# RuanJohn/Mava

Measured on AMD Instinct MI355X. Metric: env-steps/sec (whole node), ff_mappo RWARE tiny-4ag, higher is better.
Workload: dtype f32 via 2 x f16 split operands on the MFMA (3 products, f32 accumulate); 1 GPU; ff_mappo RWARE tiny-4ag-shaped synthetic obs, 4096 envs/GPU (update_batch_size=1 x num_envs=4096), rollout_length=128, ppo_epochs=4, num_minibatches=2, agents=4, obs=70/264, actions=5, one step = one PPO update = 524288 env-steps per GPU; parallelism=dp1

## Files before the change

### include/mava_hip.h

```cpp
#ifndef MAVA_HIP_H
#define MAVA_HIP_H

#include <stddef.h>
#include <stdint.h>

#ifdef __cplusplus
extern "C" {
#endif

typedef struct ihipStream_t* mava_stream_t;

const char* mava_last_error(void);
int mava_abi_version(void);

typedef struct mava_ctx mava_ctx;
enum {
  MAVA_CTX_MATMUL_MODE = 0,
  MAVA_CTX_CRITIC_AGGREGATION = 1,
  MAVA_CTX_GAE_VARIANT = 2,
  MAVA_CTX_POLICY_VARIANT = 3,
  MAVA_CTX_H2_LAUNCHES = 4,
  MAVA_CTX_TRAIN_VARIANT = 5,
  MAVA_CTX_W8_LAUNCHES = 6,
  MAVA_CTX_W1_SPLIT_FRESH = 7,
  MAVA_CTX_EXACT_TILES = 8,
  MAVA_CTX_X16_LAUNCHES = 9,
  MAVA_CTX_X16_W8_LAUNCHES = 10,
  MAVA_CTX_W8_DEFER_LAUNCHES = 11,
  MAVA_CTX_W8_AHEAD_LAUNCHES = 12
};
int mava_ctx_create(mava_ctx** out);
int mava_ctx_destroy(mava_ctx* ctx);
int mava_ctx_set(mava_ctx* ctx, int key, long value);
int mava_ctx_get(const mava_ctx* ctx, int key, long* value);

int mava_gae_f32(const mava_ctx* ctx, const float* reward, const float* value, const uint8_t* done,
                 const float* last_val, const uint8_t* last_done, int T, int N, float gamma,
                 float lambda, float* adv, float* tgt, mava_stream_t s);

int mava_permutation_i32(long n, uint64_t seed, uint64_t counter, int32_t* out, mava_stream_t s);
int mava_permutation_batched_i32(long n, uint64_t seed, uint64_t counter, int n_perm, int32_t* out, long out_stride,
                                 mava_stream_t s);

int mava_clip_adam(float* p, const float* g, float* m, float* v, int32_t* count,
                   const int* seg_off, const float* seg_lr, int n_seg, float grad_scale,
                   float max_norm, int decay, int steps_per_update, int num_updates, float b1,
                   float b2, float eps, const float* loss_sums, float vf_coef, float ent_coef,
                   float* metrics_out, mava_stream_t s);

size_t mava_ppo_finish_workspace_bytes(int Pa, int Pc);
int mava_ppo_finish_f32(mava_ctx* ctx, const float* slab_a, long stride_a, const float* slab_c, long stride_c, int n_slab,
                        int Pa, int Pc, float* g, float* p, float* m, float* v, int32_t* count, float lr_a, float lr_c,
                        float grad_scale, float max_norm, int decay, int steps_per_update, int num_updates, float b1,
                        float b2, float eps, float vf_coef, float ent_coef, float* metrics_out, int critic_din,
                        void* workspace, size_t workspace_bytes, mava_stream_t s);

int mava_slab_reduce_f32(const float* slab, int n_slab, long slab_stride, int n, int accumulate,
                         float* out, mava_stream_t s);

int mava_slab_reduce2_f32(const float* slab, int n_slab, long slab_stride, int n_main,
                          float* out_main, int n_tail, float* out_tail, int accumulate,
                          mava_stream_t s);
// ... 324 lines not shown
```

### mava_amd/_lib.py

```python
from __future__ import annotations

import ctypes as C
import os
from typing import Optional

import torch

_HERE = os.path.dirname(os.path.abspath(__file__))
LIB_PATH = os.environ.get("MAVA_LIB_PATH") or os.path.join(_HERE, "libmavahip.so")

_lib: Optional[C.CDLL] = None


class MavaHipError(RuntimeError):
    pass


vp = C.c_void_p
i32 = C.c_int
u32 = C.c_uint32
u64 = C.c_uint64
f32 = C.c_float
lng = C.c_long

# ... 106 lines not shown
             "mava_transformer_param_count_continuous": C.c_long}


def declared_symbols():
    return sorted(set(_SIGNATURES) | set(_RESTYPES))


def lib() -> C.CDLL:
    global _lib
    if _lib is None:
        if not os.path.exists(LIB_PATH):
            raise MavaHipError(
                f"{LIB_PATH} is missing: build it with `python -m mava_amd.build` "
                "(hipcc --offload-arch=gfx950). There is no CPU fallback."
            )
        _lib = C.CDLL(LIB_PATH)
        _lib.mava_last_error.restype = C.c_char_p
        _lib.mava_last_error.argtypes = []
        for name, args in _SIGNATURES.items():
            fn = getattr(_lib, name)
            fn.argtypes = args
            fn.restype = _RESTYPES.get(name, C.c_int)
    return _lib


class Ctx:

    MATMUL_MODE, CRITIC_AGGREGATION, GAE_VARIANT, POLICY_VARIANT, H2_LAUNCHES, TRAIN_VARIANT, W8_LAUNCHES, W1_SPLIT_FRESH = 0, 1, 2, 3, 4, 5, 6, 7
    EXACT_TILES = 8
    X16_LAUNCHES = 9
    X16_W8_LAUNCHES = 10
    W8_DEFER_LAUNCHES = 11
    W8_AHEAD_LAUNCHES = 12

    def __init__(self, matmul_mode: str = "f32", critic_aggregation: bool = True):
        if matmul_mode not in ("f32", "f16x2"):
            raise ValueError(f"matmul_mode must be 'f16x2' or 'f32', got {matmul_mode!r}")
        h = C.c_void_p()
        check(lib().mava_ctx_create(C.byref(h)), "mava_ctx_create")
        self.handle: Optional[int] = h.value
        self.set(self.MATMUL_MODE, 1 if matmul_mode == "f16x2" else 0)
        self.set(self.CRITIC_AGGREGATION, int(bool(critic_aggregation)))

    def set(self, key: int, value: int) -> None:
        check(lib().mava_ctx_set(self.handle, key, int(value)), "mava_ctx_set")

    def get(self, key: int) -> int:
        out = C.c_long()
        check(lib().mava_ctx_get(self.handle, key, C.byref(out)), "mava_ctx_get")
        return int(out.value)

    @property
    def matmul_mode(self) -> str:
        return "f16x2" if self.get(self.MATMUL_MODE) == 1 else "f32"

    @property
    def h2_launches(self) -> int:
        return self.get(self.H2_LAUNCHES)

    def close(self) -> None:
        if getattr(self, "handle", None) is not None and _lib is not None:
            _lib.mava_ctx_destroy(self.handle)
        self.handle = None

    def __del__(self):
        try:
# ... 41 lines not shown
```

### mava_amd/csrc/api.cpp

```cpp
#include <stdarg.h>
#include <stdio.h>
#include <string.h>

#include "common.h"
#include "ctx.h"

static thread_local char g_err[512] = "";

void mava_set_error(const char* fmt, ...) {
  va_list ap;
  va_start(ap, fmt);
  vsnprintf(g_err, sizeof(g_err), fmt, ap);
  va_end(ap);
}

extern "C" const char* mava_last_error(void) { return g_err; }

extern "C" int mava_abi_version(void) { return 4; }

enum { CTX_MATMUL_MODE = 0, CTX_CRITIC_AGGREGATION = 1, CTX_GAE_VARIANT = 2, CTX_POLICY_VARIANT = 3, CTX_H2_LAUNCHES = 4, CTX_TRAIN_VARIANT = 5, CTX_W8_LAUNCHES = 6, CTX_W1_SPLIT_FRESH = 7, CTX_EXACT_TILES = 8, CTX_X16_LAUNCHES = 9, CTX_X16_W8_LAUNCHES = 10, CTX_W8_DEFER_LAUNCHES = 11, CTX_W8_AHEAD_LAUNCHES = 12 };
static int ctx_counter_word(int key) {
  return key == CTX_W8_AHEAD_LAUNCHES ? 4 : key == CTX_W8_DEFER_LAUNCHES ? 3 : key == CTX_X16_W8_LAUNCHES ? 2 : key == CTX_X16_LAUNCHES ? 1 : 0;
}

extern "C" int mava_ctx_create(mava_ctx** out) {
  MAVA_ARG_CHECK(out != nullptr, 0, "mava_ctx_create: null output pointer");
  mava_ctx* c = new mava_ctx();
  c->matmul_mode = 0;
  c->critic_aggregation = 1;
  c->gae_variant = 0;
  c->policy_variant = 0;
  c->h2_launches = 0;
  c->train_variant = 0;
  c->w8_launches = 0;
  c->w1_split[0] = c->w1_split[1] = nullptr;
  for (int i = 0; i < 2; ++i) {
    c->w1_fresh[i] = 0;
    c->w1_key_params[i] = nullptr;
    c->w1_key_din[i] = c->w1_key_steps[i] = 0;
  }
  c->exact_tiles = nullptr;
  *out = c;
  return MAVA_OK;
}

extern "C" int mava_ctx_destroy(mava_ctx* c) {
  if (c == nullptr) return MAVA_OK;
  for (int i = 0; i < 2; ++i)
    if (c->w1_split[i] != nullptr) (void)hipFree(c->w1_split[i]);
  if (c->exact_tiles != nullptr) (void)hipFree(c->exact_tiles);
  delete c;
  return MAVA_OK;
}

extern "C" int mava_ctx_set(mava_ctx* c, int key, long value) {
  MAVA_ARG_CHECK(c != nullptr, 0, "mava_ctx_set: null context");
  switch (key) {
    case CTX_MATMUL_MODE:
      MAVA_ARG_CHECK(value == 0 || value == 1, 1, "mava_ctx_set: matmul mode %ld (0 = exact f32, 1 = f16x2)", value);
      c->matmul_mode = (int)value;
      c->w1_fresh[0] = c->w1_fresh[1] = 0;
      return MAVA_OK;
    case CTX_CRITIC_AGGREGATION: c->critic_aggregation = value ? 1 : 0; return MAVA_OK;
    case CTX_GAE_VARIANT: c->gae_variant = (int)value; return MAVA_OK;
    case CTX_POLICY_VARIANT: c->policy_variant = (int)value; return MAVA_OK;
    case CTX_H2_LAUNCHES: c->h2_launches = value; return MAVA_OK;
    case CTX_TRAIN_VARIANT: c->train_variant = (int)value; return MAVA_OK;
    case CTX_W8_LAUNCHES: c->w8_launches = value; return MAVA_OK;
    case CTX_W1_SPLIT_FRESH:
      MAVA_ARG_CHECK(value == 0, 1, "mava_ctx_set: MAVA_CTX_W1_SPLIT_FRESH can only be cleared (0) by the caller");
      c->w1_fresh[0] = c->w1_fresh[1] = 0;
      return MAVA_OK;
    case CTX_EXACT_TILES:
      MAVA_ARG_CHECK(value == 0, 1, "mava_ctx_set: MAVA_CTX_EXACT_TILES can only be reset (0) by the caller");
      if (c->exact_tiles != nullptr) {
        MAVA_HIP_CHECK(hipDeviceSynchronize());
        MAVA_HIP_CHECK(hipMemset(c->exact_tiles, 0, sizeof(unsigned long long)));
      }
      return MAVA_OK;
    case CTX_X16_LAUNCHES:
    case CTX_X16_W8_LAUNCHES:
    case CTX_W8_DEFER_LAUNCHES:
    case CTX_W8_AHEAD_LAUNCHES:
      MAVA_ARG_CHECK(value == 0, 1, "mava_ctx_set: MAVA_CTX_X16_LAUNCHES / _W8_LAUNCHES / MAVA_CTX_W8_DEFER_LAUNCHES / _AHEAD_LAUNCHES can only be reset (0) by the caller");
      if (c->exact_tiles != nullptr) {
        MAVA_HIP_CHECK(hipDeviceSynchronize());
        MAVA_HIP_CHECK(hipMemset(c->exact_tiles + ctx_counter_word(key), 0, sizeof(unsigned long long)));
      }
      return MAVA_OK;
    default: mava_set_error("mava_ctx_set: unknown key %d", key); return MAVA_EARG(2);
  }
}

extern "C" int mava_ctx_get(const mava_ctx* c, int key, long* value) {
  MAVA_ARG_CHECK(c != nullptr && value != nullptr, 0, "mava_ctx_get: null argument");
  switch (key) {
    case CTX_MATMUL_MODE: *value = c->matmul_mode; return MAVA_OK;
    case CTX_CRITIC_AGGREGATION: *value = c->critic_aggregation; return MAVA_OK;
    case CTX_GAE_VARIANT: *value = c->gae_variant; return MAVA_OK;
    case CTX_POLICY_VARIANT: *value = c->policy_variant; return MAVA_OK;
    case CTX_H2_LAUNCHES: *value = c->h2_launches; return MAVA_OK;
    case CTX_TRAIN_VARIANT: *value = c->train_variant; return MAVA_OK;
    case CTX_W8_LAUNCHES: *value = c->w8_launches; return MAVA_OK;
    case CTX_W1_SPLIT_FRESH: *value = c->w1_fresh[1]; return MAVA_OK;
    case CTX_EXACT_TILES:
    case CTX_X16_LAUNCHES:
    case CTX_X16_W8_LAUNCHES:
    case CTX_W8_DEFER_LAUNCHES:
    case CTX_W8_AHEAD_LAUNCHES: {
      unsigned long long n = 0;
      if (c->exact_tiles != nullptr) {
        MAVA_HIP_CHECK(hipDeviceSynchronize());
        MAVA_HIP_CHECK(hipMemcpy(&n, c->exact_tiles + ctx_counter_word(key), sizeof(n), hipMemcpyDeviceToHost));
      }
      *value = (long)n;
      return MAVA_OK;
    }
    default: mava_set_error("mava_ctx_get: unknown key %d", key); return MAVA_EARG(2);
  }
}
```

### mava_amd/csrc/ppo_train_h2.hip

```cpp
#include "h2_core.h"
#include "ppo_train_task.h"
#include "ctx.h"

#include <type_traits>

#ifndef MAVA_GW_DEPTH
#define MAVA_GW_DEPTH 0
#endif
#define GW_DEPTH MAVA_GW_DEPTH
#ifndef MAVA_GW_DEPTH_WIDE
#define MAVA_GW_DEPTH_WIDE 0
#endif
#ifndef MAVA_P1_EARLY_HALVES
#define MAVA_P1_EARLY_HALVES 2
#endif
#ifndef MAVA_P1_EARLY_RING
#define MAVA_P1_EARLY_RING 3
#endif

namespace {

using namespace h2;

constexpr int STATS_BLOCKS = 128;

#ifdef MAVA_STAMPS
#define STAMP_DECL unsigned long long st_prev = __builtin_readcyclecounter(), st_acc[16] = {0, 0, 0, 0, 0, 0, 0, 0, 0, 0, 0, 0, 0, 0, 0, 0};
#define STAMP(i)                                                    \
  do {                                                              \
    __builtin_amdgcn_sched_barrier(0);                              \
    const unsigned long long st_now = __builtin_readcyclecounter(); \
    st_acc[i] += st_now - st_prev;                                  \
    st_prev = st_now;                                               \
    __builtin_amdgcn_sched_barrier(0);                              \
  } while (0)
#else
#define STAMP_DECL
#define STAMP(i)
#endif

struct H2Layout {
  int h1, dz2, dz1, w2, xs, xs_plane, xs_row, dy, yp, agg, small, relu, end;
};

template <int NO, int S1, bool WIDE>
H2Layout make_h2_layout(bool actor) {
  constexpr int KT1 = (S1 + 1) / 2;
  H2Layout L;
  L.h1 = 0;
  L.dz2 = L.h1 + IMG_BYTES;
  L.dz1 = L.dz2 + IMG_BYTES;
  L.w2 = L.dz1 + IMG_BYTES;
  L.xs = L.w2 + 4 * IMG_BYTES;
  L.xs_row = 2 * 32 * KT1 + 16;
  L.xs_plane = 32 * L.xs_row;
  L.dy = L.xs + (WIDE ? 1 : 2) * 2 * L.xs_plane;
  L.yp = actor ? L.dz2 : L.dz1;
  L.agg = L.dy + (actor ? 2 * DY_PLANE : 0);
  L.small = L.agg + 8 * 33 * 4;
  L.small = (L.small + 15) & ~15;
  L.relu = L.small + (128 + 32 + 16 + 128) * 4;
  L.end = L.relu + (WIDE ? 256 * 4 : 0);
  return L;
}
constexpr int W2_PLANE = 128 * SW_ROW;
constexpr int W1_RING = 3;

template <int STEPS>
__global__ __launch_bounds__(256) void pack_w1_kernel(const float* __restrict__ P, int din, uint4* __restrict__ out, float scale) {
  pack_w1_body<STEPS>(P, din, out, threadIdx.x, scale);
}

template <int NO, int S1, bool ACTOR, bool WIDE, int XV, int ROLE, bool X16 = false>
__device__ __forceinline__ void h2_body(const TrainTask& tk, const H2Layout& L, const uint4* __restrict__ w1p, u8* lds) {
  static_assert(!WIDE || S1 % W1_RING == 0, "WIDE: S1 must be a multiple of the W1 ring depth");
  static_assert((ROLE == 0) == !WIDE, "roles 1 / 2 belong to WIDE launches");
  static_assert(!X16 || (WIDE && !ACTOR), "the f16 copy of x is read by the wide critic only");
  constexpr bool CHAIN = ROLE != 2, LOADER = ROLE != 1;
#if defined(MAVA_NO_W2_RESIDENT) || defined(MAVA_W2_RESIDENT_P4)
  constexpr bool W2_RESIDENT = false;
#else
  constexpr bool W2_RESIDENT = !WIDE && NO <= 16;
#endif
#ifdef MAVA_W2_RESIDENT_P4
  constexpr bool W2_RES4 = !WIDE && ACTOR && NO <= 16;
#else
  constexpr bool W2_RES4 = false;
#endif
  constexpr int NTHR = WIDE ? 512 : 256;
  constexpr float WS = ACTOR ? 1.0f : W_SCALE_CRITIC, WU = 1.0f / WS;
  constexpr int KT1 = (S1 + 1) / 2;
  u8* const H1I = lds + L.h1;
  u8* const DZ2I = lds + L.dz2;
  u8* const DZ1I = lds + L.dz1;
  u8* const H2I = lds + L.dz1;
  u8* const W2I = lds + L.w2;
  u8* const DYI = lds + L.dy;
  float* const YP = reinterpret_cast<float*>(lds + L.yp);
  float* const AGG = reinterpret_cast<float*>(lds + L.agg);
  float* const B2s = reinterpret_cast<float*>(lds + L.small);
  float* const B3s = B2s + 128;
  float* const misc = B3s + 32;
  float* const W3s = misc + 16;
  uint32_t* const RELU1 = reinterpret_cast<uint32_t*>(lds + L.relu);
  constexpr bool VERSIONED = WIDE && !ACTOR;
  constexpr int P1_EARLY = VERSIONED ? MAVA_P1_EARLY_HALVES * (S1 / 2) : 0;
  static_assert(MAVA_P1_EARLY_HALVES >= 0 && MAVA_P1_EARLY_HALVES <= 2, "P1_EARLY is 0, S1 / 2 or S1");
  constexpr bool EARLY = P1_EARLY > 0, EARLY_ALL = EARLY && P1_EARLY == S1;
  const int xs_row = L.xs_row, xs_plane = L.xs_plane;

  int tid = threadIdx.x & 255;
  int lane = tid & 63, w = tid >> 6, h = lane >> 5, r = lane & 31;
  int srow = tid >> 3, l8 = tid & 7;
  const int din = tk.din, no = tk.no;
  const long R = (!ACTOR && tk.agg > 1) ? (long)tk.Rb : (long)tk.Rb * tk.A;
  const float invR = 1.0f / (float)((long)tk.Rb * tk.A);
  constexpr int NPC = (32 * KT1 / XV + 7) / 8;
  constexpr int NR = NPC * XV;

  for (int i = threadIdx.x * 16; i < L.end; i += NTHR * 16) *reinterpret_cast<uint4*>(lds + i) = make_uint4(0, 0, 0, 0);
  __syncthreads();
  const float* const P = tk.params;
  const int oW2 = mlp_off_w2(din), oW3 = mlp_off_w3(din);
  if (CHAIN) {
    if (tid < 128) B2s[tid] = P[mlp_off_b2(din) + tid];
    if (tid < no) B3s[tid] = P[mlp_off_b3(din, no) + tid];
    if (!ACTOR && tid < 128) W3s[tid] = P[oW3 + tid];
    if (tid < (WIDE ? 32 : 64)) {
      const int b = tid >> 5, row = tid & 31;
      *reinterpret_cast<_Float16*>(lds + L.xs + b * 2 * xs_plane + row * xs_row + 2 * din) = (_Float16)1.0f;
    }
    {
      const int n = tid & 127, k0 = 64 * (tid >> 7);
      float carry = 0.0f;
#pragma unroll 8
      for (int k = k0; k < k0 + 64; ++k) {
        _Float16 x0, x1;
        split1_carry(P[oW2 + k * MLP_H + n] * WS, carry, x0, x1);
        const int o = sw_off(k, n >> 3) + 2 * (n & 7);
        *reinterpret_cast<_Float16*>(W2I + o) = x0;
        *reinterpret_cast<_Float16*>(W2I + W2_PLANE + o) = x1;
// ... 260 lines not shown
        cursor_advance(cs);
      }
      if (CHAIN) {
#pragma unroll
        for (int q = 0; q < NP; ++q) cursor_gather(cl[q], pl_next[q], al_next[q]);
#pragma unroll
        for (int q = 0; q < NP; ++q) cursor_advance(cl[q]);
      }
    }
  }
  __syncthreads();

  SwRow rowB = sw_row(r, h);
  SwTr trS = sw_tr(lane);
  const int i16 = lane & 15, tq = i16 >> 2, tp = i16 & 3, g1 = (lane >> 4) & 1;
  int trX = (8 * h + tq) * xs_row + 2 * (16 * g1 + 4 * tp);
  const int trD = (8 * h + tq) * DY_ROW + 2 * (16 * g1 + 4 * tp);
  SwRow w2row = sw_row(32 * w + r, h);
  int buf = 0;
  Frag w2r[(W2_RESIDENT || W2_RES4) ? 8 : 1];
  if constexpr (W2_RESIDENT) {
#pragma unroll
    for (int s = 0; s < 8; ++s) w2r[s] = sw_read_tr(W2I, W2_PLANE, trS, s, w);
  }
  if constexpr (W2_RES4) {
#pragma unroll
    for (int s = 0; s < 8; ++s) w2r[s] = sw_read_row(W2I, W2_PLANE, w2row, s);
  }

  STAMP_DECL
  bool exact = false;
  unsigned n_exact = 0;
  constexpr int ER = MAVA_P1_EARLY_RING, SB = S1 - P1_EARLY;
  constexpr int GB = P1_EARLY / 9, GC = GB + (P1_EARLY * 7) / 18;
  f32x16 eC, eL;
  Frag W1e[(EARLY && LOADER) ? ER : 1];
  auto early_fill = [&]() __attribute__((always_inline)) {
#pragma unroll
    for (int g = 0; g < ER && g < P1_EARLY; ++g) W1e[g] = w1_fetch(SB + g);
  };
  auto early_steps = [&](auto g0_tag, auto g1_tag, const u8* xsi) __attribute__((always_inline)) {
    constexpr int G0 = decltype(g0_tag)::value, G1 = decltype(g1_tag)::value;
    if constexpr (G0 < G1) {
      half8 xh = *reinterpret_cast<const half8*>(xsi + r * xs_row + 16 * h + 32 * (SB + G0));
#pragma unroll
      for (int g = G0; g < G1; ++g) {
        const half8 b = xh;
        if (g + 1 < G1) xh = *reinterpret_cast<const half8*>(xsi + r * xs_row + 16 * h + 32 * (SB + g + 1));
        if (g == 0 || SB + g == S1 / 2) {
#pragma unroll
          for (int q = 0; q < 16; ++q) {
            if (SB + g < S1 / 2) eC[q] = 0.0f; else eL[q] = 0.0f;
          }
        }
        if (SB + g < S1 / 2) {
          eC = __builtin_amdgcn_mfma_f32_32x32x16_f16(W1e[g % ER].lo, b, eC, 0, 0, 0);
          eC = __builtin_amdgcn_mfma_f32_32x32x16_f16(W1e[g % ER].hi, b, eC, 0, 0, 0);
        } else {
          eL = __builtin_amdgcn_mfma_f32_32x32x16_f16(W1e[g % ER].lo, b, eL, 0, 0, 0);
          eL = __builtin_amdgcn_mfma_f32_32x32x16_f16(W1e[g % ER].hi, b, eL, 0, 0, 0);
        }
        if (g >= 1 && g - 1 + ER < P1_EARLY) W1e[(g - 1) % ER] = w1_fetch(SB + g - 1 + ER);
        __builtin_amdgcn_sched_barrier(0);
      }
    }
  };
  uint32_t xrow_keep = 0;
  auto tile_body = [&](auto exact_tag) __attribute__((always_inline)) {
    constexpr bool EXACT = decltype(exact_tag)::value;
    static_assert(!EXACT || VERSIONED, "the exact-input loop belongs to the wide critic");
    constexpr bool XE = EXACT && EARLY;
    STAMP(14);
    const bool valid = (it * 32 + r) < R;
    const long itn = it + gridDim.x;
    const bool have_next = itn < ntiles;
    if constexpr (EXACT && LOADER && !X16) {
      if (tid == 0) xflag[tpar ^ 1] = 0u;
    }
    uint32_t xrow_next = LOADER ? stage_row(ps_next, as_next) : 0u;
    uint32_t fr_next[NP];
#pragma unroll
    for (int q = 0; q < NP; ++q) fr_next[q] = CHAIN ? ((uint32_t)pl_next[q] * Au + al_next[q]) : 0u;
    if (LOADER) asm volatile("" : "+v"(xrow_next));
    if (CHAIN) {
#pragma unroll
      for (int q = 0; q < NP; ++q) asm volatile("" : "+v"(fr_next[q]));
    }
    const u8* const XSI = lds + L.xs + (EXACT ? tpar : 2 * buf) * xs_plane;
    if constexpr (XE && LOADER) xrow_keep = xrow_next;

    f32x16 acc;
    uint32_t relu1 = 0;
    if constexpr (WIDE) asm volatile("" : "+v"(w1p_lane));
    if constexpr ((CHAIN || WIDE) && !(XE && (LOADER || EARLY_ALL))) {
#pragma unroll
    for (int q = 0; q < 16; ++q) acc[q] = 0.0f;
    if constexpr (WIDE && !CHAIN) {
#pragma unroll
      for (int s = 0; s < NW1; ++s) W1f[s] = w1_fetch(S_LO + s);
    }
    Frag xb;
    xb.hi = *reinterpret_cast<const half8*>(XSI + r * xs_row + 16 * h + 32 * S_LO);
    if constexpr (!EXACT) xb.lo = *reinterpret_cast<const half8*>(XSI + xs_plane + r * xs_row + 16 * h + 32 * S_LO);
#pragma unroll
    for (int j = 0; j < RL; ++j) {
      const Frag b = xb;
      if (j + 1 < RL) {
        xb.hi = *reinterpret_cast<const half8*>(XSI + r * xs_row + 16 * h + 32 * (S_LO + j + 1));
        if constexpr (!EXACT) xb.lo = *reinterpret_cast<const half8*>(XSI + xs_plane + r * xs_row + 16 * h + 32 * (S_LO + j + 1));
      }
      if constexpr (EXACT) {
        acc = __builtin_amdgcn_mfma_f32_32x32x16_f16(W1f[j % NW1].lo, b.hi, acc, 0, 0, 0);
        acc = __builtin_amdgcn_mfma_f32_32x32x16_f16(W1f[j % NW1].hi, b.hi, acc, 0, 0, 0);
      } else {
        acc = mfma3(W1f[j % NW1], b, acc);
      }
      if (WIDE) {
        if (j >= 1 && j - 1 + W1_RING < RL) W1f[(j - 1) % NW1] = w1_fetch(S_LO + j - 1 + W1_RING);
      }
      __builtin_amdgcn_sched_barrier(0);
    }
    }
    if constexpr (XE && EARLY_ALL && LOADER) {
#pragma unroll
      for (int q = 0; q < 16; ++q) {
        acc[q] = fmaxf((eC[q] + eL[q]) * WU, 0.0f);
        relu1 |= (acc[q] > 0.0f) ? (1u << q) : 0u;
      }
      __builtin_amdgcn_sched_barrier(0);
      issue(have_next ? xrow_next : 0u);
      __builtin_amdgcn_sched_barrier(0);
      half4 ph[4], pl[4];
      sw_write_image(H1I, r, w, h, acc, ph, pl);
      RELU1[tid] = relu1;
    }
    if constexpr (WIDE && !(XE && EARLY_ALL)) {
      float4* const xch = reinterpret_cast<float4*>(DZ2I) + (w * 4) * 64 + lane;
      if constexpr (LOADER) {
        if constexpr (XE) {
          acc = eL;
          issue(have_next ? xrow_next : 0u);
        }
#pragma unroll
        for (int g = 0; g < 4; ++g) xch[g * 64] = make_float4(acc[4 * g], acc[4 * g + 1], acc[4 * g + 2], acc[4 * g + 3]);
      }
      __syncthreads();
      if constexpr (CHAIN) {
#pragma unroll
        for (int g = 0; g < 4; ++g) {
          const float4 v = xch[g * 64];
          acc[4 * g] += v.x; acc[4 * g + 1] += v.y; acc[4 * g + 2] += v.z; acc[4 * g + 3] += v.w;
        }
      }
    }
    if constexpr (CHAIN && !(XE && EARLY_ALL)) {
    STAMP(0);
#pragma unroll
    for (int q = 0; q < 16; ++q) {
      acc[q] = fmaxf(ACTOR ? acc[q] : acc[q] * WU, 0.0f);
      relu1 |= (acc[q] > 0.0f) ? (1u << q) : 0u;
    }
    {
      half4 ph[4], pl[4];
      sw_write_image(H1I, r, w, h, acc, ph, pl);
// ... 30 lines not shown
      }
    } else if (have_next) {
      if (LOADER && !WIDE) issue(xrow_next);
      const bool more = itn + gridDim.x < ntiles;
      if (more) {
        if (LOADER) {
          cursor_gather(cs, ps_next, as_next);
          cursor_advance(cs);
        }
        if (CHAIN) {
          Cursor c_old[NP];
#pragma unroll
          for (int q = 0; q < NP; ++q) { c_old[q] = cl[q]; cursor_advance(cl[q]); }
          __builtin_amdgcn_sched_barrier(0);
#pragma unroll
          for (int q = 0; q < NP; ++q) cursor_gather(c_old[q], pl_next[q], al_next[q]);
        }
      }
      if (CHAIN) {
#pragma unroll
        for (int q = 0; q < NP; ++q) load_row((long)fr_next[q], n_act[q], n_f0[q], n_f1[q], n_m[q]);
      }
    }
    if constexpr (WIDE && CHAIN && !(XE && EARLY_ALL)) {
      __builtin_amdgcn_sched_barrier(0);
#pragma unroll
      for (int s2 = 0; s2 < NW1; ++s2) W1f[s2] = w1_fetch(S_LO + s2);
      __builtin_amdgcn_sched_barrier(0);
    }
    STAMP(2);
    __syncthreads();
    STAMP(3);
    if constexpr (XE && LOADER) {
      commit_hi(lds + L.xs + (tpar ^ 1) * xs_plane, tpar ^ 1);
      early_fill();
    }
    if constexpr (XE && EARLY_ALL && CHAIN) relu1 = RELU1[tid];

    f32x16 h2;
    uint32_t relu2 = 0;
    if constexpr (CHAIN) {
#pragma unroll
    for (int q = 0; q < 16; ++q) h2[q] = B2s[32 * w + (q & 3) + 8 * (q >> 2) + 4 * h] * WS;
    {
      Frag an;
      if constexpr (!W2_RESIDENT) an = sw_read_tr(W2I, W2_PLANE, trS, 0, w);
      Frag bn = sw_read_row(H1I, SW_PLANE, rowB, 0);
#pragma unroll
      for (int s = 0; s < 8; ++s) {
        const Frag a = W2_RESIDENT ? w2r[s] : an, b = bn;
        if (s + 1 < 8) {
          if constexpr (!W2_RESIDENT) an = sw_read_tr(W2I, W2_PLANE, trS, s + 1, w);
          bn = sw_read_row(H1I, SW_PLANE, rowB, s + 1);
        }
        h2 = mfma3(a, b, h2);
        __builtin_amdgcn_sched_barrier(0);
      }
    }
    STAMP(4);
#pragma unroll
    for (int q = 0; q < 16; ++q) {
      h2[q] = fmaxf(ACTOR ? h2[q] : h2[q] * WU, 0.0f);
      relu2 |= (h2[q] > 0.0f) ? (1u << q) : 0u;
    }
    if (!ACTOR) {
      float4 w3g[4];
#pragma unroll
      for (int g = 0; g < 4; ++g) w3g[g] = *reinterpret_cast<const float4*>(W3s + 32 * w + 4 * h + 8 * g);
// ... 1 lines not shown
#pragma unroll
      for (int q = 0; q < 16; ++q) {
        const float4 t = w3g[q >> 2];
        const float w3 = (q & 3) == 0 ? t.x : (q & 3) == 1 ? t.y : (q & 3) == 2 ? t.z : t.w;
        part = fmaf(h2[q], w3, part);
      }
      part += __shfl_xor(part, 32, 64);
      if (h == 0) YP[(w * 32 + r) * (NO + 1)] = part;
    } else {
      half4 ph[4], pl[4];
      sw_write_image(H2I, r, w, h, h2, ph, pl);
      f32x16 yacc;
#pragma unroll
      for (int q = 0; q < 16; ++q) yacc[q] = 0.0f;
#pragma unroll
      for (int s = 0; s < 2; ++s) {
        Frag b;
        b.hi = __builtin_shufflevector(ph[2 * s], ph[2 * s + 1], 0, 1, 2, 3, 4, 5, 6, 7);
        b.lo = __builtin_shufflevector(pl[2 * s], pl[2 * s + 1], 0, 1, 2, 3, 4, 5, 6, 7);
        yacc = mfma3(W3h[s], b, yacc);
      }
#pragma unroll
      for (int q = 0; q < 16; ++q) {
        const int o = (q & 3) + 8 * (q >> 2) + 4 * h;
        if ((q & 3) + 8 * (q >> 2) < NO) {
          if (o < NO) YP[(w * 32 + r) * (NO + 1) + o] = yacc[q] * W3_UNSCALE;
        }
      }
    }
    }
    STAMP(5);
    __syncthreads();
    STAMP(6);
    if constexpr (XE && LOADER) early_steps(std::integral_constant<int, 0>{}, std::integral_constant<int, GB>{}, lds + L.xs + (tpar ^ 1) * xs_plane);
    if constexpr (EXACT && LOADER && !XE) {
      commit_hi(lds + L.xs + (tpar ^ 1) * xs_plane, tpar ^ 1);
    }

    f32x16 dz;
    float dy0 = 0.0f;
    if constexpr (CHAIN) {
    if (ACTOR) {
      const float lo_c = 1.0f - tk.clip_eps, hi_c = 1.0f + tk.clip_eps;
#pragma unroll
      for (int q = 0; q < NP; ++q) {
        const int row = loss_row(q);
        const bool rvalid = (it * 32 + row) < R;
        const float* yp = YP + row * (NO + 1) + lo;
        const float y = (((yp[0] + yp[32 * (NO + 1)]) + yp[2 * 32 * (NO + 1)]) + yp[3 * 32 * (NO + 1)]) + B3s[lo];
        const bool legal = (lo < no) && (r_m[q] != 0u);
        const float z = legal ? y : -FLT_MAX;
        auto fmax_op = [](float a, float b) { return fmaxf(a, b); };
        auto add_op = [](float a, float b) { return a + b; };
        const float mx = group_allreduce<NO>(z, fmax_op);
        const float se = group_allreduce<NO>(expf(z - mx), add_op);
        const float logp = (mx == -FLT_MAX) ? ((lo < no) ? -logf((float)no) : -FLT_MAX) : z - (mx + logf(se));
        const float pr = expf(logp);
        const float ent = group_allreduce<NO>((pr > 0.0f) ? -(pr * logp) : 0.0f, add_op);
        const int act = r_act[q];
        const float lp = group_allreduce<NO>((lo == act) ? logp : 0.0f, add_op);
        const float gae = (r_f1[q] - adv_mean) * adv_rstd;
        const float ratio = expf(lp - r_f0[q]);
        const float rc = fminf(fmaxf(ratio, lo_c), hi_c);
        const float l1 = ratio * gae, l2 = rc * gae;
        const float pg = -fminf(l1, l2);
        const bool inside = (ratio >= lo_c) && (ratio <= hi_c);
// ... 131 lines not shown
      if constexpr (!W2_RES4) an = sw_read_row(W2I, W2_PLANE, w2row, 0);
      Frag bn = sw_read_row(DZ2I, SW_PLANE, rowB, 0);
#pragma unroll
      for (int s = 0; s < 8; ++s) {
        const Frag a = W2_RES4 ? w2r[s] : an, b = bn;
        if (s + 1 < 8) {
          if constexpr (!W2_RES4) an = sw_read_row(W2I, W2_PLANE, w2row, s + 1);
          bn = sw_read_row(DZ2I, SW_PLANE, rowB, s + 1);
        }
        acc = mfma3(a, b, acc);
        __builtin_amdgcn_sched_barrier(0);
      }
#pragma unroll
      for (int q = 0; q < 16; ++q) acc[q] = ((relu1 >> q) & 1u) ? (ACTOR ? acc[q] : acc[q] * WU) : 0.0f;
      half4 ph[4], pl[4];
      sw_write_image(DZ1I, r, w, h, acc, ph, pl);
    }
    if constexpr (!WIDE) {
      if constexpr (!X16) {
        if (have_next) stage_commit(false_type{}, false_type{}, lds + L.xs + (buf ^ 1) * 2 * xs_plane, xr, 0);
      }
    }
    if constexpr (XE && LOADER) early_steps(std::integral_constant<int, GC>{}, std::integral_constant<int, P1_EARLY>{}, lds + L.xs + (tpar ^ 1) * xs_plane);
    STAMP(10);
    if constexpr (!WIDE) do_gw2();
    STAMP(11);
    __syncthreads();
    STAMP(12);
    if constexpr (WIDE && CHAIN) do_gw2();
    if constexpr (LOADER) {
      constexpr int NPR = 2 * KT1;
      constexpr int D1 = WIDE ? MAVA_GW_DEPTH_WIDE : GW_DEPTH;
      if constexpr (EXACT) {
#pragma unroll
        for (int s = 0; s < 2; ++s) {
          const Frag b = sw_read_tr(DZ1I, SW_PLANE, trS, s, w);
#pragma unroll
          for (int t = 0; t < KT1; ++t) {
            const half8 a = read_tr8(XSI + trX + 16 * s * xs_row + 2 * (32 * t), xs_row);
            const f32x16 c = __builtin_amdgcn_mfma_f32_32x32x16_f16(a, b.lo, gW1[t], 0, 0, 0);
            gW1[t] = __builtin_amdgcn_mfma_f32_32x32x16_f16(a, b.hi, c, 0, 0, 0);
            if (t & 1) __builtin_amdgcn_sched_barrier(0);
          }
        }
      } else if constexpr (D1 > 0) {
        constexpr int DP = D1 < NPR ? D1 : NPR;
        const Frag b0 = sw_read_tr(DZ1I, SW_PLANE, trS, 0, w), b1 = sw_read_tr(DZ1I, SW_PLANE, trS, 1, w);
        Frag a[DP > 0 ? DP : 1];
#pragma unroll
        for (int i = 0; i < DP; ++i) a[i] = read_tr_frag(XSI + trX + 16 * (i / KT1) * xs_row + 2 * (32 * (i % KT1)), xs_plane, xs_row);
#pragma unroll
        for (int i = 0; i < NPR; ++i) {
          const Frag cur = a[i % (DP > 0 ? DP : 1)];
          if (i + DP < NPR)
            a[i % (DP > 0 ? DP : 1)] = read_tr_frag(XSI + trX + 16 * ((i + DP) / KT1) * xs_row + 2 * (32 * ((i + DP) % KT1)), xs_plane, xs_row);
          gW1[i % KT1] = mfma3(cur, (i / KT1) ? b1 : b0, gW1[i % KT1]);
          __builtin_amdgcn_sched_barrier(0);
        }
      } else {
#pragma unroll
        for (int s = 0; s < 2; ++s) {
          const Frag b = sw_read_tr(DZ1I, SW_PLANE, trS, s, w);
#pragma unroll
          for (int t = 0; t < KT1; ++t) {
            const Frag a = read_tr_frag(XSI + trX + 16 * s * xs_row + 2 * (32 * t), xs_plane, xs_row);
            gW1[t] = mfma3(a, b, gW1[t]);
            if (t & 1) __builtin_amdgcn_sched_barrier(0);
          }
        }
      }
    }
    STAMP(13);
    if constexpr (WIDE) {
      __syncthreads();
      if constexpr (EXACT) {
        if constexpr (!X16) exact = __builtin_amdgcn_readfirstlane((int)xflag[tpar ^ 1]) == 0;
        ++n_exact;
      } else {
        if constexpr (LOADER && !X16) {
          stage_commit(false_type{}, false_type{}, lds + L.xs, xr, 0);
        }
        __syncthreads();
      }
    }
    if constexpr (CHAIN) {
#pragma unroll
      for (int q = 0; q < NP; ++q) { r_act[q] = n_act[q]; r_f0[q] = n_f0[q]; r_f1[q] = n_f1[q]; r_m[q] = n_m[q]; }
    }
  };
  if constexpr (VERSIONED) {
    exact = X16 || (__builtin_amdgcn_readfirstlane((int)xflag[0]) == 0 && tk.force_xlo == 0);
    if (exact && it < ntiles) {
      if (CHAIN && tid < 32) *reinterpret_cast<_Float16*>(lds + L.xs + xs_plane + tid * xs_row + 2 * din) = (_Float16)1.0f;
    }
    if constexpr (EARLY && LOADER) {
      early_fill();
      early_steps(std::integral_constant<int, 0>{}, std::integral_constant<int, P1_EARLY>{}, lds + L.xs);
    }
    if constexpr (X16) {
      for (; it < ntiles; it += gridDim.x, tpar ^= 1) tile_body(true_type{});
    } else {
    for (; it < ntiles && exact; it += gridDim.x, tpar ^= 1) tile_body(true_type{});
    asm volatile("" : "+v"(tid), "+v"(lane), "+v"(w), "+v"(h), "+v"(r), "+v"(trS.b0), "+v"(trS.b1), "+v"(trS.q64));
    if constexpr (LOADER) asm volatile("" : "+v"(srow), "+v"(l8), "+v"(trX));
    if constexpr (CHAIN) asm volatile("" : "+v"(rowB.base), "+v"(rowB.hx), "+v"(w2row.base), "+v"(w2row.hx));
    if (n_exact != 0 && it < ntiles) {
      if constexpr (LOADER) {
        if constexpr (EARLY) {
          asm volatile("" : "+v"(xrow_keep));
          stage_issue(xrow_keep, xr);
        }
        stage_commit(false_type{}, false_type{}, lds + L.xs, xr, 0);
      }
      if (CHAIN && tid < 32) *reinterpret_cast<_Float16*>(lds + L.xs + xs_plane + tid * xs_row + 2 * din) = (_Float16)0.0f;
      __syncthreads();
    }
    if constexpr (EARLY_ALL && CHAIN) {
#pragma unroll
      for (int s = 0; s < NW1; ++s) W1f[s] = w1_fetch(S_LO + s);
    }
    }
  }
  if constexpr (!X16) {
    for (; it < ntiles; it += gridDim.x, buf ^= (WIDE ? 0 : 1)) tile_body(false_type{});
  }
#ifdef MAVA_STAMPS
  if (tk.stamps != nullptr && blockIdx.x == 0 && lane == 0) {
    for (int i = 0; i < 16; ++i) tk.stamps[((ROLE == 2 ? 4 : 0) + w) * 16 + i] = st_acc[i];
  }
#endif

  __syncthreads();
  if constexpr (VERSIONED && CHAIN) {
    if (tid == 0 && tk.exact_tiles != nullptr) atomicAdd(tk.exact_tiles, (unsigned long long)n_exact);
    if constexpr (X16) {
      if (tid == 0 && blockIdx.x == 0 && tk.x16_launches != nullptr) atomicAdd(tk.x16_launches, 1ull);
    }
  }
  float* slab = tk.slab + (long)blockIdx.x * tk.slab_stride;
  const int oB2 = mlp_off_b2(din), oB3 = mlp_off_b3(din, no);
  const int Pn = mlp_param_count(din, no);
  if constexpr (LOADER) {
#pragma unroll
    for (int t = 0; t < KT1; ++t)
#pragma unroll
      for (int q = 0; q < 16; ++q) {
        const int k = mlp_feat(t, q, h);
        if (k <= din) slab[k * MLP_H + 32 * w + r] = gW1[t][q] * invR;
      }
  }
  if constexpr (CHAIN) {
#pragma unroll
    for (int t = 0; t < 4; ++t)
#pragma unroll
      for (int q = 0; q < 16; ++q) slab[oW2 + mlp_feat(t, q, h) * MLP_H + 32 * w + r] = gW2[t][q] * invR;
#pragma unroll
    for (int q = 0; q < 16; ++q) {
      float v = ab2[q];
#pragma unroll
      for (int m = 1; m < 32; m <<= 1) v += __shfl_xor(v, m, 64);
      if (r == 0) slab[oB2 + 32 * w + (q & 3) + 8 * (q >> 2) + 4 * h] = v * invR;
    }
  }
  float* red = reinterpret_cast<float*>(lds + L.h1);
  if constexpr (!CHAIN) {
    __syncthreads();
  } else if (ACTOR) {
#pragma unroll
    for (int q = 0; q < 16; ++q) {
      const int o = (q & 3) + 8 * (q >> 2) + 4 * h;
      if (o < no) slab[oW3 + (32 * w + r) * no + o] = gW3[q] * invR;
// ... 18 lines not shown
    for (int q = 0; q < 16; ++q) {
      float v = aW3r[q];
#pragma unroll
      for (int m = 1; m < 32; m <<= 1) v += __shfl_xor(v, m, 64);
      if (r == 0) slab[oW3 + 32 * w + (q & 3) + 8 * (q >> 2) + 4 * h] = v * invR;
    }
    float v = ab3, l = loss_a;
    for (int o = 32; o > 0; o >>= 1) {
      v += __shfl_down(v, o, 64);
      l += __shfl_down(l, o, 64);
    }
    if (lane == 0) { red[2 * w] = v; red[2 * w + 1] = l; }
    __syncthreads();
    if (tid == 0) {
      slab[oB3] = (((red[0] + red[2]) + red[4]) + red[6]) * invR;
      slab[Pn] = ((red[1] + red[3]) + red[5]) + red[7];
      slab[Pn + 1] = 0.0f;
    }
  }
}

template <int NO, int S1, bool ACTOR, bool WIDE, int XV>
__global__ __launch_bounds__(WIDE ? 512 : 256, WIDE ? 2 : 1) void ppo_train_h2_kernel(TrainTask tk, H2Layout L,
                                                                                     const uint4* __restrict__ w1p) {
  extern __shared__ __attribute__((aligned(16))) u8 lds[];
  if constexpr (WIDE) {
    constexpr bool X16_CAPABLE = !ACTOR && XV == 4;
    bool x16 = false;
    if constexpr (X16_CAPABLE) {
      if (tk.x16_valid != nullptr) x16 = __builtin_amdgcn_readfirstlane((int)*tk.x16_valid) == 1;
    }
    if (X16_CAPABLE && x16) {
      if constexpr (X16_CAPABLE) {
        if (threadIdx.x < 256) {
          h2_body<NO, S1, ACTOR, WIDE, XV, 1, true>(tk, L, w1p, lds);
        } else {
          h2_body<NO, S1, ACTOR, WIDE, XV, 2, true>(tk, L, w1p, lds);
        }
      }
    } else if (threadIdx.x < 256) {
      h2_body<NO, S1, ACTOR, WIDE, XV, 1>(tk, L, w1p, lds);
    } else {
      h2_body<NO, S1, ACTOR, WIDE, XV, 2>(tk, L, w1p, lds);
    }
  } else {
    h2_body<NO, S1, ACTOR, WIDE, XV, 0>(tk, L, w1p, lds);
  }
}

int ctx_counters(mava_ctx* ctx, hipStream_t s) {
  if (ctx->exact_tiles == nullptr) {
    void* word = nullptr;
    MAVA_HIP_CHECK(hipMalloc(&word, 5 * sizeof(unsigned long long)));
    ctx->exact_tiles = static_cast<unsigned long long*>(word);
    MAVA_HIP_CHECK(hipMemsetAsync(word, 0, 5 * sizeof(unsigned long long), s));
  }
  return MAVA_OK;
}

template <int NO, int S1, bool ACTOR, bool WIDE, int XV>
int launch_h2(mava_ctx* ctx, const TrainTask& tk, int n_slab, hipStream_t s) {
  const H2Layout L = make_h2_layout<NO, S1, WIDE>(ACTOR);
  MAVA_ARG_CHECK(L.end <= 163840, 8, "ppo_train_h2: %d bytes of LDS exceed the 160 KiB of a CU", L.end);
  static bool attr_set = false;
  if (!attr_set) {
    MAVA_HIP_CHECK(hipFuncSetAttribute((const void*)ppo_train_h2_kernel<NO, S1, ACTOR, WIDE, XV>,
                                       hipFuncAttributeMaxDynamicSharedMemorySize, L.end));
    attr_set = true;
  }
  const uint4* w1p = nullptr;
  if (WIDE) {
    void*& slot = ctx->w1_split[ACTOR ? 0 : 1];
    if (slot == nullptr) MAVA_HIP_CHECK(hipMalloc(&slot, W1_SPLIT_BYTES));
    uint4* const buf = static_cast<uint4*>(slot);
    const int kind = ACTOR ? 0 : 1;
    int& fresh = ctx->w1_fresh[kind];
    const bool keyed = ctx->w1_key_params[kind] == tk.params && ctx->w1_key_din[kind] == tk.din && ctx->w1_key_steps[kind] == S1;
    if (!(fresh && keyed)) {
      hipLaunchKernelGGL((pack_w1_kernel<S1>), dim3(1), dim3(256), 0, s, tk.params, tk.din, buf, ACTOR ? 1.0f : W_SCALE_CRITIC);
      MAVA_LAUNCH_CHECK();
    }
    fresh = 0;
    w1p = buf;
    const int rc = ctx_counters(ctx, s);
    if (rc != MAVA_OK) return rc;
  }
  TrainTask tkl = tk;
  tkl.exact_tiles = WIDE ? ctx->exact_tiles : nullptr;
  const bool x16_ok = WIDE && !ACTOR && XV == 4 && tk.x16 != nullptr && tk.x16_valid != nullptr && tk.din % 8 == 0 &&
                      (uintptr_t)tk.x16 % 16 == 0 && tk.force_xlo == 0 && (tk.x16_ld == 0 || tk.x16_ld == tk.din);
  if (!x16_ok) { tkl.x16 = nullptr; tkl.x16_valid = nullptr; }
  tkl.x16_launches = x16_ok ? ctx->exact_tiles + 1 : nullptr;
  g_train_last_instance = train_instance_id(2, ACTOR, false, WIDE, NO, S1, XV);
  hipLaunchKernelGGL((ppo_train_h2_kernel<NO, S1, ACTOR, WIDE, XV>), dim3(n_slab), dim3(WIDE ? 512 : 256), L.end, s, tkl, L,
                     w1p);
  MAVA_LAUNCH_CHECK();
  return MAVA_OK;
}

template <int NO, int S1, bool ACTOR, bool WIDE>
int dispatch_xv(mava_ctx* ctx, const TrainTask& tk, int n_slab, hipStream_t s) {
  const uintptr_t a = (uintptr_t)tk.x;
  if constexpr (WIDE) {
    if (tk.din % 4 == 0 && a % 16 == 0) return launch_h2<NO, S1, ACTOR, WIDE, 4>(ctx, tk, n_slab, s);
  } else {
    if (tk.din % 2 == 0 && a % 8 == 0) return launch_h2<NO, S1, ACTOR, WIDE, 2>(ctx, tk, n_slab, s);
  }
  return launch_h2<NO, S1, ACTOR, WIDE, 1>(ctx, tk, n_slab, s);
}

template <int NO, bool ACTOR>
int dispatch_s1(mava_ctx* ctx, const TrainTask& tk, int n_slab, hipStream_t s) {
  const int s1 = (tk.din + 1 + 15) / 16;
  switch (s1) {
#ifndef MAVA_FAST_BUILD
    case 1: return dispatch_xv<NO, 1, ACTOR, false>(ctx, tk, n_slab, s);
    case 2: return dispatch_xv<NO, 2, ACTOR, false>(ctx, tk, n_slab, s);
    case 3: return dispatch_xv<NO, 3, ACTOR, false>(ctx, tk, n_slab, s);
    case 4: return dispatch_xv<NO, 4, ACTOR, false>(ctx, tk, n_slab, s);
    case 6: return dispatch_xv<NO, 6, ACTOR, false>(ctx, tk, n_slab, s);
    case 7: case 8: case 9: case 10: case 11: case 12: return dispatch_xv<NO, 12, ACTOR, true>(ctx, tk, n_slab, s);
#endif
    case 5: return dispatch_xv<NO, 5, ACTOR, false>(ctx, tk, n_slab, s);
    case 13: case 14: case 15: case 16: case 17: case 18: return dispatch_xv<NO, 18, ACTOR, true>(ctx, tk, n_slab, s);
    default: return 1;
  }
}

}

static int h2_dispatch(mava_ctx* ctx, const TrainTask& tk, int n_slab, bool actor, hipStream_t s) {
  if (actor) {
    if (tk.action_f != nullptr) return 1;
    if (tk.no <= 8) return dispatch_s1<8, true>(ctx, tk, n_slab, s);
#ifndef MAVA_FAST_BUILD
    if (tk.no <= 16) return dispatch_s1<16, true>(ctx, tk, n_slab, s);
    return dispatch_s1<32, true>(ctx, tk, n_slab, s);
#else
    return 1;
#endif
  }
  return dispatch_s1<1, false>(ctx, tk, n_slab, s);
}

int mava_train_h2_launch(mava_ctx* ctx, const TrainTask& tk_in, int n_slab, bool actor, hipStream_t s) {
  TrainTask tk = tk_in;
  tk.force_xlo = (ctx->train_variant & 2) != 0;
  tk.no_defer = (ctx->train_variant & 4) != 0;
  tk.no_ahead = (ctx->train_variant & 8) != 0;
  if ((ctx->train_variant & 1) == 0) {
    if (tk.x16 != nullptr && tk.x16_valid != nullptr) {
      const int rcc = ctx_counters(ctx, s);
      if (rcc != MAVA_OK) return rcc;
      tk.x16_launches = ctx->exact_tiles + 2;
      tk.defer_launches = ctx->exact_tiles + 3;
      tk.ahead_launches = ctx->exact_tiles + 4;
    }
    const int rc8 = mava_train_w8_launch(tk, n_slab, actor, s);
    if (rc8 <= 0) {
      if (rc8 == 0) { ++ctx->h2_launches; ++ctx->w8_launches; }
      return rc8;
    }
  }
  const int rc = h2_dispatch(ctx, tk, n_slab, actor, s);
  if (rc == 0) ++ctx->h2_launches;
  return rc;
}
```

### mava_amd/csrc/ppo_train_task.h

```cpp
#pragma once
#include <stdint.h>

#include "common.h"

struct TrainTask {
  const float* params;
  const float* x;
  int din, no, xshare, xv;
  int A;
  int agg;
  const int32_t* idx;
  long idx_base;
  int Rb;
  const uint8_t* mask;
  const int32_t* action;
  const float* action_f;
  uint32_t seed_lo, seed_hi, ent_step, row_offset;
  float min_scale;
  const float* old_logp;
  const float* adv;
  const double* stats;
  const float* old_value;
  const float* targets;
  float clip_eps, ent_coef, vf_coef;
  float* slab;
  long slab_stride;
  unsigned long long* stamps;
  int force_xlo;
  unsigned long long* exact_tiles;
  const _Float16* x16;
  const uint32_t* x16_valid;
  unsigned long long* x16_launches;
  int x16_ld;
  int no_defer;
  unsigned long long* defer_launches;
  int no_ahead;
  unsigned long long* ahead_launches;
};

struct mava_ctx;
int mava_train_w8_launch(const TrainTask& tk, int n_slab, bool actor, hipStream_t s);
int mava_train_h2_launch(mava_ctx* ctx, const TrainTask& tk, int n_slab, bool actor, hipStream_t s);

extern int g_train_last_instance;
constexpr int train_instance_id(int family, bool actor, bool cont, bool wide, int no, int k, int xv) {
  return family * 1000000 + ((actor ? 1 : 0) + (cont ? 2 : 0) + (wide ? 4 : 0)) * 100000 + no * 1000 + k * 10 + xv;
}
```

Before: 88.09 million env-steps/s.

## Defer tail of exact dW1 products into next tile's loader phase for wide critic

```diff
diff --git a/include/mava_hip.h b/include/mava_hip.h
--- a/include/mava_hip.h
+++ b/include/mava_hip.h
@@ -27,7 +27,8 @@
   MAVA_CTX_X16_LAUNCHES = 9,
   MAVA_CTX_X16_W8_LAUNCHES = 10,
   MAVA_CTX_W8_DEFER_LAUNCHES = 11,
-  MAVA_CTX_W8_AHEAD_LAUNCHES = 12
+  MAVA_CTX_W8_AHEAD_LAUNCHES = 12,
+  MAVA_CTX_WIDE_DEFER_LAUNCHES = 13
 };
 int mava_ctx_create(mava_ctx** out);
 int mava_ctx_destroy(mava_ctx* ctx);
diff --git a/mava_amd/_lib.py b/mava_amd/_lib.py
--- a/mava_amd/_lib.py
+++ b/mava_amd/_lib.py
@@ -162,6 +162,7 @@
     X16_W8_LAUNCHES = 10
     W8_DEFER_LAUNCHES = 11
     W8_AHEAD_LAUNCHES = 12
+    WIDE_DEFER_LAUNCHES = 13
 
     def __init__(self, matmul_mode: str = "f32", critic_aggregation: bool = True):
         if matmul_mode not in ("f32", "f16x2"):
diff --git a/mava_amd/csrc/api.cpp b/mava_amd/csrc/api.cpp
--- a/mava_amd/csrc/api.cpp
+++ b/mava_amd/csrc/api.cpp
@@ -18,9 +18,9 @@
 
 extern "C" int mava_abi_version(void) { return 4; }
 
-enum { CTX_MATMUL_MODE = 0, CTX_CRITIC_AGGREGATION = 1, CTX_GAE_VARIANT = 2, CTX_POLICY_VARIANT = 3, CTX_H2_LAUNCHES = 4, CTX_TRAIN_VARIANT = 5, CTX_W8_LAUNCHES = 6, CTX_W1_SPLIT_FRESH = 7, CTX_EXACT_TILES = 8, CTX_X16_LAUNCHES = 9, CTX_X16_W8_LAUNCHES = 10, CTX_W8_DEFER_LAUNCHES = 11, CTX_W8_AHEAD_LAUNCHES = 12 };
+enum { CTX_MATMUL_MODE = 0, CTX_CRITIC_AGGREGATION = 1, CTX_GAE_VARIANT = 2, CTX_POLICY_VARIANT = 3, CTX_H2_LAUNCHES = 4, CTX_TRAIN_VARIANT = 5, CTX_W8_LAUNCHES = 6, CTX_W1_SPLIT_FRESH = 7, CTX_EXACT_TILES = 8, CTX_X16_LAUNCHES = 9, CTX_X16_W8_LAUNCHES = 10, CTX_W8_DEFER_LAUNCHES = 11, CTX_W8_AHEAD_LAUNCHES = 12, CTX_WIDE_DEFER_LAUNCHES = 13 };
 static int ctx_counter_word(int key) {
-  return key == CTX_W8_AHEAD_LAUNCHES ? 4 : key == CTX_W8_DEFER_LAUNCHES ? 3 : key == CTX_X16_W8_LAUNCHES ? 2 : key == CTX_X16_LAUNCHES ? 1 : 0;
+  return key == CTX_WIDE_DEFER_LAUNCHES ? 5 : key == CTX_W8_AHEAD_LAUNCHES ? 4 : key == CTX_W8_DEFER_LAUNCHES ? 3 : key == CTX_X16_W8_LAUNCHES ? 2 : key == CTX_X16_LAUNCHES ? 1 : 0;
 }
 
 extern "C" int mava_ctx_create(mava_ctx** out) {
@@ -82,7 +82,8 @@
     case CTX_X16_W8_LAUNCHES:
     case CTX_W8_DEFER_LAUNCHES:
     case CTX_W8_AHEAD_LAUNCHES:
-      MAVA_ARG_CHECK(value == 0, 1, "mava_ctx_set: MAVA_CTX_X16_LAUNCHES / _W8_LAUNCHES / MAVA_CTX_W8_DEFER_LAUNCHES / _AHEAD_LAUNCHES can only be reset (0) by the caller");
+    case CTX_WIDE_DEFER_LAUNCHES:
+      MAVA_ARG_CHECK(value == 0, 1, "mava_ctx_set: MAVA_CTX_X16_LAUNCHES / _W8_LAUNCHES / MAVA_CTX_W8_DEFER_LAUNCHES / _AHEAD_LAUNCHES / MAVA_CTX_WIDE_DEFER_LAUNCHES can only be reset (0) by the caller");
       if (c->exact_tiles != nullptr) {
         MAVA_HIP_CHECK(hipDeviceSynchronize());
         MAVA_HIP_CHECK(hipMemset(c->exact_tiles + ctx_counter_word(key), 0, sizeof(unsigned long long)));
@@ -107,7 +108,8 @@
     case CTX_X16_LAUNCHES:
     case CTX_X16_W8_LAUNCHES:
     case CTX_W8_DEFER_LAUNCHES:
-    case CTX_W8_AHEAD_LAUNCHES: {
+    case CTX_W8_AHEAD_LAUNCHES:
+    case CTX_WIDE_DEFER_LAUNCHES: {
       unsigned long long n = 0;
       if (c->exact_tiles != nullptr) {
         MAVA_HIP_CHECK(hipDeviceSynchronize());
diff --git a/mava_amd/csrc/ppo_train_h2.hip b/mava_amd/csrc/ppo_train_h2.hip
--- a/mava_amd/csrc/ppo_train_h2.hip
+++ b/mava_amd/csrc/ppo_train_h2.hip
@@ -16,6 +16,15 @@
 #endif
 #ifndef MAVA_P1_EARLY_RING
 #define MAVA_P1_EARLY_RING 3
+#endif
+#ifndef MAVA_WIDE_DEFER_STEPS
+#define MAVA_WIDE_DEFER_STEPS 8
+#endif
+#ifndef MAVA_WIDE_DEFER_STEPS_12
+#define MAVA_WIDE_DEFER_STEPS_12 6
+#endif
+#ifndef MAVA_WIDE_GATHER_BEHIND_A
+#define MAVA_WIDE_GATHER_BEHIND_A 0
 #endif
 
 namespace {
@@ -64,6 +73,7 @@
   return L;
 }
 constexpr int W2_PLANE = 128 * SW_ROW;
+constexpr int wide_defer_steps(int s1) { return s1 == 18 ? MAVA_WIDE_DEFER_STEPS : s1 == 12 ? MAVA_WIDE_DEFER_STEPS_12 : 0; }
 constexpr int W1_RING = 3;
 
 template <int STEPS>
@@ -71,11 +81,12 @@
   pack_w1_body<STEPS>(P, din, out, threadIdx.x, scale);
 }
 
-template <int NO, int S1, bool ACTOR, bool WIDE, int XV, int ROLE, bool X16 = false>
+template <int NO, int S1, bool ACTOR, bool WIDE, int XV, int ROLE, bool X16 = false, bool DEFER_T = false>
 __device__ __forceinline__ void h2_body(const TrainTask& tk, const H2Layout& L, const uint4* __restrict__ w1p, u8* lds) {
   static_assert(!WIDE || S1 % W1_RING == 0, "WIDE: S1 must be a multiple of the W1 ring depth");
   static_assert((ROLE == 0) == !WIDE, "roles 1 / 2 belong to WIDE launches");
   static_assert(!X16 || (WIDE && !ACTOR), "the f16 copy of x is read by the wide critic only");
+  static_assert(!DEFER_T || X16, "the deferred-dW1 schedule belongs to the bodies that stage from the f16 copy");
   constexpr bool CHAIN = ROLE != 2, LOADER = ROLE != 1;
 #if defined(MAVA_NO_W2_RESIDENT) || defined(MAVA_W2_RESIDENT_P4)
   constexpr bool W2_RESIDENT = false;
@@ -107,6 +118,9 @@
   constexpr int P1_EARLY = VERSIONED ? MAVA_P1_EARLY_HALVES * (S1 / 2) : 0;
   static_assert(MAVA_P1_EARLY_HALVES >= 0 && MAVA_P1_EARLY_HALVES <= 2, "P1_EARLY is 0, S1 / 2 or S1");
   constexpr bool EARLY = P1_EARLY > 0, EARLY_ALL = EARLY && P1_EARLY == S1;
+  constexpr int DW = (DEFER_T && EARLY_ALL) ? wide_defer_steps(S1) : 0;
+  constexpr bool DEFER = DW > 0;
+  static_assert(DW >= 0 && DW <= KT1, "only products of the tile's second 16 rows are deferred");
   const int xs_row = L.xs_row, xs_plane = L.xs_plane;
 
   int tid = threadIdx.x & 255;
@@ -433,7 +447,7 @@
   bool exact = false;
   unsigned n_exact = 0;
   constexpr int ER = MAVA_P1_EARLY_RING, SB = S1 - P1_EARLY;
-  constexpr int GB = P1_EARLY / 9, GC = GB + (P1_EARLY * 7) / 18;
+  constexpr int GB = DEFER ? 0 : P1_EARLY / 9, GC = DEFER ? P1_EARLY / 2 : GB + (P1_EARLY * 7) / 18;
   f32x16 eC, eL;
   Frag W1e[(EARLY && LOADER) ? ER : 1];
   auto early_fill = [&]() __attribute__((always_inline)) {
@@ -463,6 +477,24 @@
         }
         if (g >= 1 && g - 1 + ER < P1_EARLY) W1e[(g - 1) % ER] = w1_fetch(SB + g - 1 + ER);
         __builtin_amdgcn_sched_barrier(0);
+      }
+    }
+  };
+  auto dw1_exact = [&](auto p0_tag, auto p1_tag, const u8* xsi) __attribute__((always_inline)) {
+    constexpr int P0 = decltype(p0_tag)::value, P1 = decltype(p1_tag)::value;
+#pragma unroll
+    for (int s = 0; s < 2; ++s) {
+      if (P0 < (s + 1) * KT1 && s * KT1 < P1) {
+        const Frag b = sw_read_tr(DZ1I, SW_PLANE, trS, s, w);
+#pragma unroll
+        for (int t = 0; t < KT1; ++t) {
+          if (s * KT1 + t >= P0 && s * KT1 + t < P1) {
+            const half8 a = read_tr8(xsi + trX + 16 * s * xs_row + 2 * (32 * t), xs_row);
+            const f32x16 c = __builtin_amdgcn_mfma_f32_32x32x16_f16(a, b.lo, gW1[t], 0, 0, 0);
+            gW1[t] = __builtin_amdgcn_mfma_f32_32x32x16_f16(a, b.hi, c, 0, 0, 0);
+            if (t & 1) __builtin_amdgcn_sched_barrier(0);
+          }
+        }
       }
     }
   };
@@ -528,9 +560,11 @@
         acc[q] = fmaxf((eC[q] + eL[q]) * WU, 0.0f);
         relu1 |= (acc[q] > 0.0f) ? (1u << q) : 0u;
       }
-      __builtin_amdgcn_sched_barrier(0);
-      issue(have_next ? xrow_next : 0u);
-      __builtin_amdgcn_sched_barrier(0);
+      if constexpr (!(DEFER && MAVA_WIDE_GATHER_BEHIND_A)) {
+        __builtin_amdgcn_sched_barrier(0);
+        issue(have_next ? xrow_next : 0u);
+        __builtin_amdgcn_sched_barrier(0);
+      }
       half4 ph[4], pl[4];
       sw_write_image(H1I, r, w, h, acc, ph, pl);
       RELU1[tid] = relu1;
@@ -627,8 +661,16 @@
     __syncthreads();
     STAMP(3);
     if constexpr (XE && LOADER) {
-      commit_hi(lds + L.xs + (tpar ^ 1) * xs_plane, tpar ^ 1);
-      early_fill();
+      if constexpr (DEFER) {
+        if constexpr (MAVA_WIDE_GATHER_BEHIND_A) {
+          issue(have_next ? xrow_next : 0u);
+          __builtin_amdgcn_sched_barrier(0);
+        }
+        dw1_exact(std::integral_constant<int, 2 * KT1 - DW>{}, std::integral_constant<int, 2 * KT1>{}, lds + L.xs + (tpar ^ 1) * xs_plane);
+      } else {
+        commit_hi(lds + L.xs + (tpar ^ 1) * xs_plane, tpar ^ 1);
+        early_fill();
+      }
     }
     if constexpr (XE && EARLY_ALL && CHAIN) relu1 = RELU1[tid];
 
@@ -696,6 +738,11 @@
     STAMP(5);
     __syncthreads();
     STAMP(6);
+    if constexpr (XE && LOADER && DEFER) {
+      early_fill();
+      __builtin_amdgcn_sched_barrier(0);
+      commit_hi(lds + L.xs + (tpar ^ 1) * xs_plane, tpar ^ 1);
+    }
     if constexpr (XE && LOADER) early_steps(std::integral_constant<int, 0>{}, std::integral_constant<int, GB>{}, lds + L.xs + (tpar ^ 1) * xs_plane);
     if constexpr (EXACT && LOADER && !XE) {
       commit_hi(lds + L.xs + (tpar ^ 1) * xs_plane, tpar ^ 1);
@@ -893,17 +940,7 @@
       constexpr int NPR = 2 * KT1;
       constexpr int D1 = WIDE ? MAVA_GW_DEPTH_WIDE : GW_DEPTH;
       if constexpr (EXACT) {
-#pragma unroll
-        for (int s = 0; s < 2; ++s) {
-          const Frag b = sw_read_tr(DZ1I, SW_PLANE, trS, s, w);
-#pragma unroll
-          for (int t = 0; t < KT1; ++t) {
-            const half8 a = read_tr8(XSI + trX + 16 * s * xs_row + 2 * (32 * t), xs_row);
-            const f32x16 c = __builtin_amdgcn_mfma_f32_32x32x16_f16(a, b.lo, gW1[t], 0, 0, 0);
-            gW1[t] = __builtin_amdgcn_mfma_f32_32x32x16_f16(a, b.hi, c, 0, 0, 0);
-            if (t & 1) __builtin_amdgcn_sched_barrier(0);
-          }
-        }
+        dw1_exact(std::integral_constant<int, 0>{}, std::integral_constant<int, NPR - DW>{}, XSI);
       } else if constexpr (D1 > 0) {
         constexpr int DP = D1 < NPR ? D1 : NPR;
         const Frag b0 = sw_read_tr(DZ1I, SW_PLANE, trS, 0, w), b1 = sw_read_tr(DZ1I, SW_PLANE, trS, 1, w);
@@ -960,6 +997,9 @@
     }
     if constexpr (X16) {
       for (; it < ntiles; it += gridDim.x, tpar ^= 1) tile_body(true_type{});
+      if constexpr (DEFER && LOADER) {
+        if (n_exact != 0) dw1_exact(std::integral_constant<int, 2 * KT1 - DW>{}, std::integral_constant<int, 2 * KT1>{}, lds + L.xs + (tpar ^ 1) * xs_plane);
+      }
     } else {
     for (; it < ntiles && exact; it += gridDim.x, tpar ^= 1) tile_body(true_type{});
     asm volatile("" : "+v"(tid), "+v"(lane), "+v"(w), "+v"(h), "+v"(r), "+v"(trS.b0), "+v"(trS.b1), "+v"(trS.q64));
@@ -998,6 +1038,9 @@
       if (tid == 0 && blockIdx.x == 0 && tk.x16_launches != nullptr) atomicAdd(tk.x16_launches, 1ull);
     }
   }
+  if constexpr (DEFER && LOADER) {
+    if (tid == 0 && blockIdx.x == 0 && tk.wide_defer_launches != nullptr) atomicAdd(tk.wide_defer_launches, 1ull);
+  }
   float* slab = tk.slab + (long)blockIdx.x * tk.slab_stride;
   const int oB2 = mlp_off_b2(din), oB3 = mlp_off_b3(din, no);
   const int Pn = mlp_param_count(din, no);
@@ -1082,8 +1125,11 @@
     }
     if (X16_CAPABLE && x16) {
       if constexpr (X16_CAPABLE) {
+        constexpr bool DEFER_CAPABLE = wide_defer_steps(S1) > 0;
         if (threadIdx.x < 256) {
           h2_body<NO, S1, ACTOR, WIDE, XV, 1, true>(tk, L, w1p, lds);
+        } else if (DEFER_CAPABLE && tk.no_wide_defer == 0) {
+          if constexpr (DEFER_CAPABLE) h2_body<NO, S1, ACTOR, WIDE, XV, 2, true, true>(tk, L, w1p, lds);
         } else {
           h2_body<NO, S1, ACTOR, WIDE, XV, 2, true>(tk, L, w1p, lds);
         }
@@ -1101,9 +1147,9 @@
 int ctx_counters(mava_ctx* ctx, hipStream_t s) {
   if (ctx->exact_tiles == nullptr) {
     void* word = nullptr;
-    MAVA_HIP_CHECK(hipMalloc(&word, 5 * sizeof(unsigned long long)));
+    MAVA_HIP_CHECK(hipMalloc(&word, 6 * sizeof(unsigned long long)));
     ctx->exact_tiles = static_cast<unsigned long long*>(word);
-    MAVA_HIP_CHECK(hipMemsetAsync(word, 0, 5 * sizeof(unsigned long long), s));
+    MAVA_HIP_CHECK(hipMemsetAsync(word, 0, 6 * sizeof(unsigned long long), s));
   }
   return MAVA_OK;
 }
@@ -1141,6 +1187,7 @@
                       (uintptr_t)tk.x16 % 16 == 0 && tk.force_xlo == 0 && (tk.x16_ld == 0 || tk.x16_ld == tk.din);
   if (!x16_ok) { tkl.x16 = nullptr; tkl.x16_valid = nullptr; }
   tkl.x16_launches = x16_ok ? ctx->exact_tiles + 1 : nullptr;
+  tkl.wide_defer_launches = x16_ok ? ctx->exact_tiles + 5 : nullptr;
   g_train_last_instance = train_instance_id(2, ACTOR, false, WIDE, NO, S1, XV);
   hipLaunchKernelGGL((ppo_train_h2_kernel<NO, S1, ACTOR, WIDE, XV>), dim3(n_slab), dim3(WIDE ? 512 : 256), L.end, s, tkl, L,
                      w1p);
@@ -1198,6 +1245,7 @@
   tk.force_xlo = (ctx->train_variant & 2) != 0;
   tk.no_defer = (ctx->train_variant & 4) != 0;
   tk.no_ahead = (ctx->train_variant & 8) != 0;
+  tk.no_wide_defer = (ctx->train_variant & 16) != 0;
   if ((ctx->train_variant & 1) == 0) {
     if (tk.x16 != nullptr && tk.x16_valid != nullptr) {
       const int rcc = ctx_counters(ctx, s);
diff --git a/mava_amd/csrc/ppo_train_task.h b/mava_amd/csrc/ppo_train_task.h
--- a/mava_amd/csrc/ppo_train_task.h
+++ b/mava_amd/csrc/ppo_train_task.h
@@ -36,6 +36,8 @@
   unsigned long long* defer_launches;
   int no_ahead;
   unsigned long long* ahead_launches;
+  int no_wide_defer;
+  unsigned long long* wide_defer_launches;
 };
 
 struct mava_ctx;
```

Result: no change. 88.87 million env-steps/s (median of 6 runs) (+0.9%).
